# zijinxuxu/PDFNet

Measured on AMD Instinct MI355X. Metric: train-step images/sec @256x256 RGB-D B=32, higher is better.
Workload: dtype f32

## Files before the change

### include/pdfnet_hip.h

```cpp
#ifndef PDFNET_HIP_H
#define PDFNET_HIP_H
#ifdef __cplusplus
extern "C" {
#endif

#define PDF_E_BADARG (-1)
#define PDF_E_WORKSPACE (-2)
#define PDF_ACT_NONE 0
#define PDF_ACT_RELU 1
#define PDF_ACT_LRELU01 2


int pdf_linear_fwd(const float* x, const float* w, const float* bias, float* y,
                   int M, int N, int K, int ldx, int ldw, int ldy, int act, void* stream);
int pdf_linear_bwd_weight(const float* x, const float* dy, float* dw, float* db, float* ws, long ws_floats,
                          int M, int N, int K, int ldx, int lddy, int accumulate, void* stream);
long pdf_wgrad_workspace_floats(int M, int NI, int NJ);
int pdf_init(void);
int pdf_debug_init_device(void);
int pdf_debug_kernel_timing(int on);
int pdf_set_stats_output(float* part, long cap_floats);
long pdf_stats_result_tiles(void);
long pdf_stats_result_rows(void);
int pdf_set_bn_tile_stats(const float* part, long tiles, long rows_per_tile);
// ... 234 lines not shown
typedef struct PdfCallOpts {
    const void* op0_bf16; const void* op1_bf16;
    void* out_bf16;
    const void* bn_x_bf16;
    float* stats_out; long stats_cap;
    long stats_tiles; long stats_rows;
    const float* tile_stats; long tile_n; long tile_rows;
    const float* in_scale; const float* in_shift;
    const void* op1_bf16_t;
    float* ws; long ws_floats;
    const float* wino_v;
} PdfCallOpts;
long pdf_conv2d_winograd_v_offset(int N, int H, int W, int Cin, int Cout, int KH, int KW, int stride, int pad);
int pdf_linear_fwd_x(const float* x, const float* w, const float* bias, float* y, int M, int N, int K, int ldx, int ldw, int ldy, int act, void* stream, PdfCallOpts* opts);
int pdf_linear_fwd_pair_x(const float* x, const float* w0, const float* w1, const float* b0, const float* b1, float* y, int M, int N, int K, int ldx, int ldw, int ldy, int act, void* stream, PdfCallOpts* opts);
int pdf_linear_bwd_data_x(const float* dy, const float* w, float* dx, int M, int N, int K, int lddy, int ldw, int lddx, void* stream, PdfCallOpts* opts);
int pdf_linear_bwd_data_pair_x(const float* dy, const float* w0, const float* w1, float* dx, int M, int N, int K, int lddy, int ldw, int lddx, void* stream, PdfCallOpts* opts);
int pdf_conv2d_fwd_x(const float* x, const float* w, const float* bias, float* y, int N, int H, int W, int Cin, int ldx, int Cout, int KH, int KW, int stride, int pad, int OH, int OW, int ldy, int act, void* stream, PdfCallOpts* opts);
int pdf_conv2d_bwd_data_x(const float* dy, const float* w, float* dx, int N, int H, int W, int Cin, int lddx, int Cout, int KH, int KW, int stride, int pad, int OH, int OW, int lddy, void* stream, PdfCallOpts* opts);
int pdf_conv2d_bwd_data_add_x(const float* dy, const float* w, float* dx, int N, int H, int W, int Cin, int lddx, int Cout, int KH, int KW, int stride, int pad, int OH, int OW, int lddy, void* stream, PdfCallOpts* opts);
int pdf_linear_bwd_weight_x(const float* x, const float* dy, float* dw, float* db, float* ws, long ws_floats, int M, int N, int K, int ldx, int lddy, int accumulate, void* stream, PdfCallOpts* opts);
int pdf_linear_bwd_weight_pair_x(const float* x, const float* dy, float* dw0, float* dw1, float* db0, float* db1, float* ws, long ws_floats, int M, int N, int K, int ldx, int lddy, int accumulate, void* stream, PdfCallOpts* opts);
int pdf_conv2d_bwd_weight_x(const float* x, const float* dy, float* dw, float* db, float* ws, long ws_floats, int N, int H, int W, int Cin, int ldx, int Cout, int KH, int KW, int stride, int pad, int OH, int OW, int lddy, int accumulate, void* stream, PdfCallOpts* opts);
int pdf_deconv2d_fwd_x(const float* x, const float* w, const float* bias, float* y, int N, int H, int W, int Cin, int ldx, int Cout, int KH, int KW, int stride, int pad, int OH, int OW, int ldy, void* stream, PdfCallOpts* opts);
int pdf_deconv2d_bwd_data_x(const float* dy, const float* w, float* dx, int N, int H, int W, int Cin, int lddx, int Cout, int KH, int KW, int stride, int pad, int OH, int OW, int lddy, void* stream, PdfCallOpts* opts);
int pdf_deconv2d_bwd_weight_x(const float* x, const float* dy, float* dw, float* ws, long ws_floats, int N, int H, int W, int Cin, int ldx, int Cout, int KH, int KW, int stride, int pad, int OH, int OW, int lddy, int accumulate, void* stream, PdfCallOpts* opts);
int pdf_bn_train_fwd_x(const float* x, int ldx, int C, long R, const float* gamma, const float* beta, float* running_mean, float* running_var, float momentum, float eps, const float* res, int ldr, int relu, float* y, int ldy, float* save_mean, float* save_rstd, float* scale, float* shift, float* ws, void* stream, PdfCallOpts* opts);
int pdf_bn_train_bwd_x(const float* dy, int lddy, const float* y, int ldy, int relu, const float* x, int ldx, const float* save_mean, const float* save_rstd, const float* gamma, const float* scale, const float* shift, int C, long R, float* dx, int lddx, float* dres, int lddr, float* dgamma, float* dbeta, int accumulate, float* ws, void* stream, PdfCallOpts* opts);
int pdf_bn_relu_maxk_fwd_x(const float* y, int ldy, int C, long R, int K, const float* gamma, const float* beta, float* running_mean, float* running_var, float momentum, float eps, int training, float* out, int ldo, int* arg, float* save_mean, float* save_rstd, float* scale, float* shift, float* ws, void* stream, PdfCallOpts* opts);
int pdf_l2norm_cat_fwd_x(int nparts, const float* const* x, const int* C, const float* const* w, float eps, long R, float* y, int ldy, float* const* norm, void* stream, PdfCallOpts* opts);
long pdf_conv2d_winograd_workspace_floats(int N, int H, int W, int Cin, int Cout, int KH, int KW, int stride, int pad, int backward);
int pdf_debug_armed_slots(void);
int pdf_debug_callopts_size(void);

int pdf_x3_split(const float* x, void* out, long n, long cs, void* stream);
long pdf_deconv2d_x3_workspace_floats(int N, int H, int W, int Cin, int Cout, int KH, int KW, int stride, int pad, int backward);
int pdf_set_x3_mode(int mode);
int pdf_stream_create(void** out, int priority, int* lo, int* hi);
int pdf_debug_x3_mode(void);
int pdf_debug_x3_stamps(unsigned long long* out);
int pdf_x3_batched_gemm_nt(const void* A3, long csA, const void* B3, long csB, float* C, int batch, long gsA, long gsB, long gsC, int M, int N, int K, int variant, int nprod, void* stream);
int pdf_batched_gemm_nt(const float* A, const float* B, float* C, int batch, long gsA, long gsB, long gsC, int M, int N, int K, void* stream);
int pdf_x3_batched_gemm_tn(const void* P3, long csP, const void* Q3, long csQ, float* slab, int batch, long gsP, long gsQ, int M, int NI, int NJ, int splits, int variant, int nprod, void* stream);
int pdf_batched_gemm_tn(const float* P, const float* Q, float* slab, int batch, long gsP, long gsQ, int M, int NI, int NJ, int splits, void* stream);

typedef struct PdfMeshLin { const float* w[2]; const float* b[2]; } PdfMeshLin;
typedef struct PdfMeshLN { const float* g[2]; const float* b[2]; } PdfMeshLN;
typedef struct PdfMeshGcn { PdfMeshLin fc1, fc2, sc; PdfMeshLN n2, n3; unsigned long long seed; } PdfMeshGcn;
typedef struct PdfMeshAttn {
    PdfMeshLN ln; PdfMeshLin q, k, v, fc; PdfMeshLN ffln; PdfMeshLin f1, f2;
    unsigned long long seed_att, seed_z, seed_t, seed_x;
} PdfMeshAttn;
typedef struct PdfMeshLinG { float* w[2]; float* b[2]; } PdfMeshLinG;
typedef struct PdfMeshLNG { float* g[2]; float* b[2]; } PdfMeshLNG;
typedef struct PdfMeshGcnG { PdfMeshLinG fc1, fc2, sc; PdfMeshLNG n2, n3; } PdfMeshGcnG;
typedef struct PdfMeshAttnG { PdfMeshLNG ln; PdfMeshLinG q, k, v, fc; PdfMeshLNG ffln; PdfMeshLinG f1, f2; } PdfMeshAttnG;
typedef struct PdfMeshLevel {
    int level, B, training, cin0;
    float p;
    const unsigned long long* step;
    const float* x;
    float* out;
    const int* ell_col[2]; const float* ell_val[2]; const int* ell_colT[2]; const float* ell_valT[2]; int ell_w;
    PdfMeshGcn gcn[4];
    PdfMeshAttn self_, cross;
    float* tape;
    float* qkv;
    const float* dout;
    float* dx;
    float* gtape;
    PdfMeshGcnG ggcn[4]; PdfMeshAttnG gself, gcross;
    float* wg_ws; long wg_ws_floats;
} PdfMeshLevel;
long pdf_mesh_tape_floats(int level, int B);
long pdf_mesh_gtape_floats(int level, int B);
int pdf_mesh_level_fwd(const PdfMeshLevel* a, void* stream);
int pdf_mesh_level_bwd(const PdfMeshLevel* a, void* stream, void* side_stream);
int pdf_mesh_level_fwd_bf16(const PdfMeshLevel* a, void* stream);
int pdf_mesh_level_bwd_bf16(const PdfMeshLevel* a, void* stream, void* side_stream);
int pdf_mesh_level_fwd_x3(const PdfMeshLevel* a, void* stream);
int pdf_mesh_level_bwd_x3(const PdfMeshLevel* a, void* stream, void* side_stream);
int pdf_debug_mesh_level_size(void);

typedef struct PdfMeshLoss {
    const float* vp; const float* v2p; const float* hd3; const float* hd2; const float* r;
    const float* vgt[2]; const float* jgt[2]; const float* v2gt[2]; const float* lmsgt[2];
    const long long* ind; const float* K; const float* valid;
    const float* reg[2]; const long long* faces; const long long* perm[2];
    int B, Fc, size, down;
    float* part;
    float* out;
    float coef[12];
    const float* gmp;
    int edge_grad;
    float* dvp; float* dv2p; float* dhd3; float* dhd2; float* dr;
} PdfMeshLoss;
int pdf_mesh_loss_fwd(const PdfMeshLoss* a, void* stream);
int pdf_mesh_loss_bwd(const PdfMeshLoss* a, void* stream);
int pdf_debug_mesh_loss_size(void);
int pdf_debug_mesh_stamps(unsigned long long* out);

#ifdef __cplusplus
}
#endif
#endif
```

### pdfnet_amd/build.py

```python
import os
import subprocess
import sys
from concurrent.futures import ThreadPoolExecutor

HERE = os.path.dirname(os.path.abspath(__file__))
CSRC = os.path.join(HERE, "csrc")
LIB = os.path.join(HERE, "libpdfnet_hip.so")
INCLUDE = os.path.join(HERE, "..", "include")
SOURCES = ["gemm.hip", "gemm_dma.hip", "gemm_x3.hip", "winograd.hip", "gemm_bf16.hip", "pointops.hip", "norm.hip", "elementwise.hip", "graph.hip", "meshdec.hip", "meshdec_bf16.hip", "meshdec_x3.hip", "mano.hip", "frontend.hip", "loss.hip", "metrics.hip", "icp.hip", "meshcloud.hip", "penetration.hip", "silhouette.hip", "render.hip", "safused.hip"]
FLAGS = ["--offload-arch=gfx950", "-O3", "-fPIC", "-std=c++17", "-fvisibility=hidden", "-Wno-unused-result", "-I" + INCLUDE]


def _stale(target, deps):
    if not os.path.exists(target):
        return True
    t = os.path.getmtime(target)
    return any(os.path.getmtime(d) > t for d in deps)


def build(force=False, verbose=True):
    hipcc = os.environ.get("HIPCC", "/opt/rocm/bin/hipcc")
    hdrs = [os.path.join(CSRC, "common.h"), os.path.join(CSRC, "gemm_common.h"), os.path.join(CSRC, "gemm_internal.h"), os.path.join(CSRC, "svd3.h"), os.path.join(CSRC, "icp_common.h"), os.path.join(INCLUDE, "pdfnet_hip.h")]
    objs, jobs = [], []
    for s in SOURCES:
        src = os.path.join(CSRC, s)
        obj = os.path.join(CSRC, s.replace(".hip", ".o"))
        objs.append(obj)
        deps = [src] + hdrs + ([os.path.join(CSRC, "meshdec.hip")] if s in ("meshdec_bf16.hip", "meshdec_x3.hip") else [])
        if force or _stale(obj, deps):
            jobs.append([hipcc] + FLAGS + ["-c", src, "-o", obj])

    def run(cmd):
        if verbose:
            print(" ".join(cmd), flush=True)
        subprocess.check_call(cmd)
    with ThreadPoolExecutor(max_workers=4) as ex:
        list(ex.map(run, jobs))
    if force or jobs or _stale(LIB, objs):
        run([hipcc, "--offload-arch=gfx950", "-shared", "-fPIC", "-o", LIB] + objs)
    return LIB


if __name__ == "__main__":
    print(build(force="--force" in sys.argv))
```

### pdfnet_amd/functional.py

```python
import ctypes
import torch
from torch.autograd import Function

from . import hip
from .hip import ptr, ptr_at, stream

ACT_NONE, ACT_RELU, ACT_LRELU = 0, 1, 2
import os as _os

_byref = ctypes.byref
_CallOpts = hip.CallOpts
USE_SIDE_STREAMS = _os.environ.get("PDFNET_SIDE_STREAMS", "1") != "0"
_side = {}


def _record(obj, stream_):
    if torch.is_tensor(obj):
        obj.record_stream(stream_)
        s16 = getattr(obj, '_pdf_bf16', None)
        if s16 is not None:
            s16.record_stream(stream_)
    elif isinstance(obj, (list, tuple)):
        for o in obj:
            _record(o, stream_)
# ... 2646 lines not shown
                getattr(getattr(dst, k), wb)[hnd] = ptr(g)
        cur = stream()
        direct = all(g is None for g in grads)
        with wgrad_stream(direct, x, tape, qkv, gtape, ws, dout, params=tensors):
            _mesh_entry(L, 'bwd')(_byref(a), cur, stream())
        ctx.keep = ctx.args = None
        return (dx, None, None) + tuple(grads)


def mesh_level(layer, x):
    tensors, _ = _mesh_param_list(layer)
    return _MeshLevel.apply(x, layer, layer.training, *tensors)


def mesh_level_ok(layer, x):
    if not (MESH_FUSED and x.is_cuda and (MESH_FUSED_BF16 or not _GEMM_BF16) and x.dim() == 4 and x.shape[0] == 2 and x.dtype == torch.float32):
        return False
    level = {63: 0, 126: 1, 252: 2}.get(x.shape[2])
    return (level is not None and x.shape[3] == 2 * (256 >> level) and len(layer.graph_left.GCN_blocks) == 4 and layer.attn.n_heads == 4
            and layer.graph_left.GCN_blocks[0].fc1.weight.shape[0] == (256 >> level) and x.shape[1] <= 2048)


MESH_LOSS_FUSED = _os.environ.get("PDFNET_MESH_LOSS_FUSED", "1") != "0"
MESH_LOSS_TERMS = ('verts2d_loss', 'norm_loss', 'edge_loss', 'gcn_2d_loss', 'root_loss', 'verts_loss', 'abs_verts_loss', 'gcn_loss',
                   'abs_joints_loss', 'joints2d_loss', 'joints_loss', 'bone_direc_loss')


class _MeshLoss(Function):

    @staticmethod
    def forward(ctx, vp, v2p, hd3, hd2, r, gt, consts, size, down, edge_grad, coefs):
        hip.require_gpu(vp)
        vp, v2p, hd3, hd2, r = (t.contiguous() for t in (vp, v2p, hd3, hd2, r))
        B = vp.shape[1]
        if vp.shape[2:] != (778, 3) or hd3.shape[2:] != (252, 3):
            raise ValueError("pdfnet_amd: mesh_loss wants the decoder's 778- and 252-vertex meshes")
        a = hip.MeshLoss()
        keep = [vp, v2p, hd3, hd2, r]
        for k, t in (('vp', vp), ('v2p', v2p), ('hd3', hd3), ('hd2', hd2), ('r', r)):
            setattr(a, k, ptr(t))
        for k in ('vgt', 'jgt', 'v2gt', 'lmsgt'):
            for i in (0, 1):
                t = gt[k][i].contiguous()
                keep.append(t)
                getattr(a, k)[i] = ptr(t)
        for k in ('ind', 'K', 'valid'):
            t = gt[k].contiguous()
            keep.append(t)
            setattr(a, k, ptr(t))
        regs, faces, perms = consts
        a.reg[0], a.reg[1] = ptr(regs[0]), ptr(regs[1])
        a.faces = ptr(faces)
        a.perm[0], a.perm[1] = ptr(perms[0]), ptr(perms[1])
        a.B, a.Fc, a.size, a.down, a.edge_grad = B, faces.shape[1], int(size), int(down), 1 if edge_grad else 0
        for i, c in enumerate(coefs):
            a.coef[i] = float(c)
        part = torch.empty((2, B, 12), dtype=torch.float32, device=vp.device)
        out = torch.empty(4 + 9 * B, dtype=torch.float32, device=vp.device)
        a.part, a.out = ptr(part), ptr(out)
        _L().pdf_mesh_loss_fwd(_byref(a), stream())
        ctx.args, ctx.keep = a, keep + [regs, faces, perms, part]
        terms = out[:4 + 8 * B]
        ctx.mark_non_differentiable(terms)
        return out[4 + 8 * B:], terms

    @staticmethod
    def backward(ctx, g, _):
        a = ctx.args
        vp, v2p, hd3, hd2, r = ctx.keep[:5]
        g = g.contiguous()
        dvp, dv2p, dhd3, dhd2, dr = (torch.empty_like(t) for t in (vp, v2p, hd3, hd2, r))
        a.gmp = ptr(g)
        a.dvp, a.dv2p, a.dhd3, a.dhd2, a.dr = ptr(dvp), ptr(dv2p), ptr(dhd3), ptr(dhd2), ptr(dr)
        _L().pdf_mesh_loss_bwd(_byref(a), stream())
        return dvp, dv2p, dhd3, dhd2, dr, None, None, None, None, None, None


def mesh_loss(vp, v2p, hd3, hd2, r, gt, consts, size, down, edge_grad, coefs):
    mp, terms = _MeshLoss.apply(vp, v2p, hd3, hd2, r, gt, consts, size, down, edge_grad, tuple(coefs))
    B = vp.shape[1]
    d = {k: terms[i] for i, k in enumerate(MESH_LOSS_TERMS[:4])}
    d.update({k: terms[4 + i * B:4 + (i + 1) * B] for i, k in enumerate(MESH_LOSS_TERMS[4:])})
    return mp, d
```

### pdfnet_amd/hip.py

```python
import ctypes
import os
import re

import torch

_HERE = os.path.dirname(os.path.abspath(__file__))
LIB_PATH = os.environ.get("PDFNET_HIP_LIB") or os.path.join(_HERE, "libpdfnet_hip.so")
HEADER_PATH = os.path.join(_HERE, "..", "include", "pdfnet_hip.h")

_CT = {"int": ctypes.c_int, "long": ctypes.c_long, "float": ctypes.c_float,
       "unsigned long long": ctypes.c_ulonglong}


def _text(path):
    return re.sub(r"/\*.*?\*/", "", open(path).read(), flags=re.S)


def parse_header(path=HEADER_PATH):
    protos = {}
    for m in re.finditer(r"\b(int|long)\s+(pdf_\w+)\s*\(([^)]*)\)\s*;", _text(path)):
        ret, name, args = m.group(1), m.group(2), m.group(3)
        types = []
        for a in args.split(","):
            a = " ".join(a.split())
            if a in ("", "void"):
                continue
            if "*" in a:
                types.append(ctypes.c_void_p)
            else:
                base = a.rsplit(" ", 1)[0]
                types.append(_CT[base])
        protos[name] = (_CT[ret], types)
    return protos


def parse_structs(path=HEADER_PATH):
    txt, structs = _text(path), {}
    for m in re.finditer(r"typedef\s+struct\s+(\w+)\s*\{([^{}]*)\}\s*\1\s*;", txt):
        fields = []
        for decl in filter(None, (" ".join(d.split()) for d in m.group(2).split(";"))):
            try:
                first, *more = decl.split(",")
                base, star, name, dim = re.fullmatch(r"(?:const )?([\w ]+?) ?(\*?) ?(\w+)(?:\[(\d+)\])?", first).groups()
                ct = ctypes.c_void_p if star else _CT.get(base) or structs[base]
                names = [(name, dim)] + [re.fullmatch(r" ?(\w+)(?:\[(\d+)\])?", d).groups() for d in more]
                if star and more:
                    raise KeyError(decl)
            except (AttributeError, KeyError):
                raise ImportError("pdfnet_amd: %s: cannot bind field `%s` of %s" % (path, decl, m.group(1)))
            fields += [(n, ct * int(d) if d else ct) for n, d in names]
        structs[m.group(1)] = type(m.group(1), (ctypes.Structure,), {"_fields_": fields})
    if len(structs) != len(re.findall(r"\b(?:struct|union)\b[^;(]*\{", txt)):
        raise ImportError("pdfnet_amd: %s has a struct / union this binding cannot parse" % path)
    return structs


STRUCTS = parse_structs()
CallOpts, MeshLevel, MeshLoss = (STRUCTS[n] for n in ("PdfCallOpts", "PdfMeshLevel", "PdfMeshLoss"))


class _Lib:
    def __init__(self):
        if not os.path.exists(LIB_PATH):
            raise ImportError(
                "pdfnet_amd: %s is missing -- build it with `python -m pdfnet_amd.build` "
                "(hipcc --offload-arch=gfx950). There is no CPU or PyTorch fallback." % LIB_PATH)
        self.cdll = ctypes.CDLL(LIB_PATH)
        self.protos = parse_header()
        for name, (ret, args) in self.protos.items():
            fn = getattr(self.cdll, name)
            fn.restype = ret
            fn.argtypes = args
        for cls, fn in ((CallOpts, "pdf_debug_callopts_size"), (MeshLoss, "pdf_debug_mesh_loss_size"), (MeshLevel, "pdf_debug_mesh_level_size")):
            if getattr(self.cdll, fn)() != ctypes.sizeof(cls):
                raise ImportError("pdfnet_amd: %s of %s has %d bytes, this binding's has %d -- rebuild the library"
                                  % (cls.__name__, LIB_PATH, getattr(self.cdll, fn)(), ctypes.sizeof(cls)))

    def __getattr__(self, name):
        fn = getattr(self.cdll, name)
        is_status = self.protos[name][0] is ctypes.c_int and not name.startswith("pdf_debug_")

        def call(*args):
            rc = fn(*args)
            if is_status and rc != 0:
                raise RuntimeError("libpdfnet_hip: %s failed with code %d" % (name, rc))
            if _tape is not None and is_status:
                _tape.append((call, args))
            return rc
        setattr(self, name, call)
        return call


_lib = None
_tape = None


def lib():
    global _lib
    if _lib is None:
        _lib = _Lib()
        if torch.cuda.is_available():
            lr = os.environ.get("LOCAL_RANK")
            if lr is not None and torch.cuda.device_count() > 1 and int(lr) != torch.cuda.current_device():
                _lib = None
                raise RuntimeError("pdfnet_amd: LOCAL_RANK=%s but the current device is cuda:%d -- call torch.cuda.set_device(LOCAL_RANK) "
                                   "(trains.base_trainer.init_distributed) before the first pdfnet_amd call" % (lr, torch.cuda.current_device()))
            _lib.pdf_init()
    return _lib


def check_device(dev):
    L = lib()
    have = L.pdf_debug_init_device()
    idx = dev.index if dev.index is not None else torch.cuda.current_device()
    if have >= 0 and have != idx:
        raise RuntimeError("pdfnet_amd: libpdfnet_hip was initialised on cuda:%d, the model lives on cuda:%d (one process per GPU)" % (have, idx))


_raw_stream = getattr(torch._C, "_cuda_getCurrentRawStream", None)
_raw_device = getattr(torch._C, "_cuda_getDevice", None)


def stream():
    if _raw_stream is not None and _raw_device is not None:
        return _raw_stream(_raw_device())
    return torch.cuda.current_stream().cuda_stream


def ptr(t):
    return t.data_ptr() if t is not None else None


def ptr_at(t, elements):
    return t.data_ptr() + elements * t.element_size()


def require_gpu(*tensors):
    for t in tensors:
        if t is not None and not t.is_cuda:
            raise RuntimeError("pdfnet_amd ops run only on the GPU (HIP); got a %s tensor. "
                               "There is no CPU fallback in the product path." % t.device)
# ... 1 lines not shown
```

### pdfnet_amd/networks/intaghand_decoder.py

```python
import os

import numpy as np
import torch
import torch.nn as nn

from .. import functional as F
from .layers import Conv2d, Embedding, LayerNorm, Linear, xavier_

_DATA = os.path.join(os.path.dirname(os.path.abspath(__file__)), "..", "data", "gcn_core.npz")
IMG_SIZE = 384


def _csr_to_ell(indptr, indices, data, V):
    width = int(np.diff(indptr).max())
    col = np.zeros((V, width), np.int32)
    val = np.zeros((V, width), np.float32)
    for v in range(V):
        a, b = indptr[v], indptr[v + 1]
        col[v, :b - a] = indices[a:b]
        val[v, :b - a] = data[a:b]
    return col, val


def load_graph_constants():
# ... 165 lines not shown
        self.position_embeddings = Embedding(V, cin)
        self.graph_left = GraphLayer(cin, cout, ellL, n, drop)
        self.graph_right = GraphLayer(cin, cout, ellR, n, drop)
        self.img_ex_left = img_ex(img_size, img_c, 6, grid_c, cout, heads, drop)
        self.img_ex_right = img_ex(img_size, img_c, 6, grid_c, cout, heads, drop)
        self.attn = inter_attn(cout, heads, drop)

    def forward(self, x):
        x = x + self.position_embeddings.weight
        if F.mesh_level_ok(self, x):
            return F.mesh_level(self, x)
        blocks = list(zip(self.graph_left.GCN_blocks, self.graph_right.GCN_blocks))
        for i, (bl, br) in enumerate(blocks):
            x = gcn_block_pair(bl, br, x, relu_out=i != len(blocks) - 1)
        return self.attn(x)


class DualGraph(nn.Module):
    def __init__(self, layers):
        super().__init__()
        self.layers = nn.ModuleList(layers)

    def forward(self, x):
        last = len(self.layers) - 1
        for i, layer in enumerate(self.layers):
            x = layer(x)
            if i != last:
                x = x.repeat_interleave(2, dim=2)
        return x


def projection_batch(scale, trans2d, pts, img_size):
    s = (scale * img_size).view(-1, 1, 1)
    t = (trans2d * img_size / 2 + img_size / 2).unsqueeze(1)
    return s * pts[..., :2] + t


class decoder(nn.Module):
    def __init__(self, opt, dropout=0.05, num_attn_heads=4):
        super().__init__()
        g = load_graph_constants()
        self.register_buffer('dense_coor', g['dense_coor'].clone())
        for h in ('left', 'right'):
            self.register_buffer('graph_perm_' + h, g['perm_' + h].clone(), persistent=False)
            self.register_buffer('graph_perm_reverse_' + h, g['perm_rev_' + h].clone(), persistent=False)
        self.converter = {h: GCN_vert_convert(self, h) for h in ('left', 'right')}
        cin, cout = opt.GCN_IN_DIM, opt.GCN_OUT_DIM
        layers = []
        for i, V in enumerate((63, 126, 252)):
            layers.append(DualGraphLayer(V, cin[i], cout[i], g['ell_left'][i], g['ell_right'][i], opt.graph_layer_num,
                                         [12, 24, 48][i], opt.DECONV_DIMS[i], opt.IMG_DIMS[i], num_attn_heads, dropout))
        self.dual_gcn = DualGraph(layers)
        d0 = cin[0] - 3
        self.gf_layer_left = nn.Sequential(Linear(1024, d0), LayerNorm(d0))
        self.gf_layer_right = nn.Sequential(Linear(1024, d0), LayerNorm(d0))
        self.unsample_layer = Linear(252, 778, bias=False)
        self.unsample_layer.weight.data.copy_(g['upsample'])
        self.coord_head = Linear(cout[-1], 3)
        self.avg_head = Linear(252, 1)
        self.params_head = Linear(cout[-1], 3)
        self.root_head = Linear(cout[-1], 3)
        for m in (self.gf_layer_left, self.gf_layer_right, self.coord_head, self.avg_head, self.params_head, self.root_head):
            xavier_(m)
        self._pe_key, self._pe = None, None

    def get_converter(self):
        return self.converter

    def hand_pe(self):
        key = (self.dense_coor._version, self.dense_coor.device)
        if self._pe_key != key:
            with torch.no_grad():
                c = (self.dense_coor * 2 - 1).unsqueeze(0)
                self._pe = torch.stack([self.converter[h].vert_to_GCN(c).view(1, 63, 16, 3).mean(2) for h in ('left', 'right')])
            self._pe_key = key
        return self._pe

    def forward(self, gl, gr):
        bs = gl.shape[0]
        g = torch.stack((gl, gr))
        f = _ln2(self.gf_layer_left[1], self.gf_layer_right[1], _lin2(self.gf_layer_left[0], self.gf_layer_right[0], g))
        x = torch.cat([f.unsqueeze(2).expand(-1, -1, 63, -1), self.hand_pe().expand(-1, bs, -1, -1)], -1)
        x = self.dual_gcn(x)
        t = self.avg_head(x.transpose(2, 3))[..., 0]
        p = self.params_head(t)
        rt = self.root_head(t)
        c3 = self.coord_head(x)
        up3 = self.unsample_layer(c3.transpose(2, 3)).transpose(2, 3).contiguous()
        sc, tr = p[..., 0], p[..., 1:]
        c2 = projection_batch(sc.reshape(-1), tr.reshape(-1, 2), c3.reshape(2 * bs, -1, 3), IMG_SIZE).view(2, bs, -1, 2)
        up2 = projection_batch(sc.reshape(-1), tr.reshape(-1, 2), up3.reshape(2 * bs, -1, 3), IMG_SIZE).view(2, bs, -1, 2)
        hands = ('left', 'right')
        scale = {h: sc[i] for i, h in enumerate(hands)}
        trans2d = {h: tr[i] for i, h in enumerate(hands)}
        root = {h: rt[i] for i, h in enumerate(hands)}
        v3 = {h: c3[i] for i, h in enumerate(hands)}
        v2 = {h: c2[i] for i, h in enumerate(hands)}
        result = {'verts3d': {h: up3[i] for i, h in enumerate(hands)}, 'verts2d': {h: up2[i] for i, h in enumerate(hands)}}
        other = {'verts3d_MANO_list': {'left': [], 'right': []}, 'verts2d_MANO_list': {'left': [], 'right': []}}
        for hand in hands:
            for key, src in (('verts3d_MANO_list', v3), ('verts2d_MANO_list', v2)):
                other[key][hand].append(self.converter[hand].GCN_to_vert(src[hand].repeat_interleave(4, dim=1)))
        return (result, {'scale': scale, 'trans2d': trans2d, 'root': root},
                [{'verts3d': v3, 'verts2d': v2}], other)


def load_decoder(opt, encoder_info=None):
    return decoder(opt, dropout=0.05, num_attn_heads=4)
```

Baseline: 718.7.

## Fuse decoder tail heads, upsample and projection into custom HIP kernels

Replaces the decoder tail (avg head, params/root/coord heads, 252→778 upsample, and both 2D projections) with one forward kernel per hand-batch item, plus a fused backward kernel and a finish kernel that reduces weight gradients across the batch. It targets the many small launches and intermediate tensors of the original chain of linear layers and transposes. In exchange, shapes are hardcoded (252 vertices, 64 channels, 778 upsampled), and the per-block backward uses large shared memory with one block per hand-batch item, so the grid is only 64 blocks.

Measured after the change: 721.2 (median of 6 runs). Within noise of the previous version (+0.4%).

```diff
diff --git a/include/pdfnet_hip.h b/include/pdfnet_hip.h
--- a/include/pdfnet_hip.h
+++ b/include/pdfnet_hip.h
@@ -340,6 +340,17 @@
 int pdf_mesh_level_bwd_x3(const PdfMeshLevel* a, void* stream, void* side_stream);
 int pdf_debug_mesh_level_size(void);
 
+#define PDF_MESH_TAIL_PART 840
+int pdf_mesh_tail_fwd(int B, float img_size, const float* x, const float* avg_w, const float* avg_b, const float* par_w, const float* par_b,
+                      const float* root_w, const float* root_b, const float* coord_w, const float* coord_b, const float* up_w,
+                      float* t, float* p, float* rt, float* c3, float* up3, float* c2, float* up2, void* stream);
+int pdf_mesh_tail_bwd(int B, float img_size, const float* x, const float* t, const float* p, const float* c3, const float* up3,
+                      const float* avg_w, const float* par_w, const float* root_w, const float* coord_w, const float* up_w,
+                      const float* dp, const float* drt, const float* dc3, const float* dup3, const float* dc2, const float* dup2,
+                      float* dx, float* gup, float* part,
+                      float* g_avg_w, float* g_avg_b, float* g_par_w, float* g_par_b, float* g_root_w, float* g_root_b, float* g_coord_w, float* g_coord_b,
+                      float* g_up_w, int overwrite, void* stream);
+
 typedef struct PdfMeshLoss {
     const float* vp; const float* v2p; const float* hd3; const float* hd2; const float* r;
     const float* vgt[2]; const float* jgt[2]; const float* v2gt[2]; const float* lmsgt[2];
diff --git a/pdfnet_amd/build.py b/pdfnet_amd/build.py
--- a/pdfnet_amd/build.py
+++ b/pdfnet_amd/build.py
@@ -7,7 +7,7 @@
 CSRC = os.path.join(HERE, "csrc")
 LIB = os.path.join(HERE, "libpdfnet_hip.so")
 INCLUDE = os.path.join(HERE, "..", "include")
-SOURCES = ["gemm.hip", "gemm_dma.hip", "gemm_x3.hip", "winograd.hip", "gemm_bf16.hip", "pointops.hip", "norm.hip", "elementwise.hip", "graph.hip", "meshdec.hip", "meshdec_bf16.hip", "meshdec_x3.hip", "mano.hip", "frontend.hip", "loss.hip", "metrics.hip", "icp.hip", "meshcloud.hip", "penetration.hip", "silhouette.hip", "render.hip", "safused.hip"]
+SOURCES = ["gemm.hip", "gemm_dma.hip", "gemm_x3.hip", "winograd.hip", "gemm_bf16.hip", "pointops.hip", "norm.hip", "elementwise.hip", "graph.hip", "meshdec.hip", "meshdec_bf16.hip", "meshdec_x3.hip", "meshglue.hip", "mano.hip", "frontend.hip", "loss.hip", "metrics.hip", "icp.hip", "meshcloud.hip", "penetration.hip", "silhouette.hip", "render.hip", "safused.hip"]
 FLAGS = ["--offload-arch=gfx950", "-O3", "-fPIC", "-std=c++17", "-fvisibility=hidden", "-Wno-unused-result", "-I" + INCLUDE]
 
 
diff --git a/pdfnet_amd/csrc/meshglue.hip b/pdfnet_amd/csrc/meshglue.hip
--- /dev/null
+++ b/pdfnet_amd/csrc/meshglue.hip
@@ -0,0 +1,354 @@
+#include "common.h"
+
+#define MT_T 1024
+#define MT_V 252
+#define MT_C 64
+#define MT_U 778
+#define MT_LDX 65
+#define MT_PART PDF_MESH_TAIL_PART
+#define MT_P_CW 0
+#define MT_P_CB 192
+#define MT_P_PW 195
+#define MT_P_PB 387
+#define MT_P_RW 390
+#define MT_P_RB 582
+#define MT_P_AW 585
+#define MT_P_AB 837
+#define MT_P_END 838
+static_assert(MT_P_END <= MT_PART, "PDF_MESH_TAIL_PART is too small");
+
+#define MT_FWD_SMEM (MT_V * MT_LDX + 1024 + 1024 + 64 + 192 + 8)
+#define MT_BWD_SMEM (MT_V * MT_LDX + 16 * MT_V * 3 + 1024 + MT_U * 4 + 64 + 64 + 192 + 64)
+
+struct MeshTail {
+    int B;
+    float img_size;
+    const float* x;
+    const float *avg_w, *avg_b, *par_w, *par_b, *root_w, *root_b, *coord_w, *coord_b, *up_w;
+    float *t, *p, *rt, *c3, *up3, *c2, *up2;
+    const float *dp, *drt, *dc3, *dup3, *dc2, *dup2;
+    float *dx, *gup, *part;
+    float *g_avg_w, *g_avg_b, *g_par_w, *g_par_b, *g_root_w, *g_root_b, *g_coord_w, *g_coord_b, *g_up_w;
+    int overwrite;
+};
+
+__device__ __forceinline__ void mt_load_x(const float* __restrict__ x, float* xs, int tid) {
+    for (int i = tid; i < MT_V * MT_C / 4; i += MT_T) {
+        const float4 v = reinterpret_cast<const float4*>(x)[i];
+        float* d = xs + (i >> 4) * MT_LDX + (i & 15) * 4;
+        d[0] = v.x; d[1] = v.y; d[2] = v.z; d[3] = v.w;
+    }
+}
+
+__global__ __launch_bounds__(MT_T, 1) void mesh_tail_fwd_kernel(const MeshTail a) {
+    extern __shared__ float smem[];
+    float* xs = smem;
+    float* red = xs + MT_V * MT_LDX;
+    float* c3s = red + 1024;
+    float* ts = c3s + 1024;
+    float* wcs = ts + 64;
+    float* ps = wcs + 192;
+    const int tid = threadIdx.x, lane = tid & 63, w = tid >> 6;
+    const long hb = blockIdx.x;
+    mt_load_x(a.x + hb * MT_V * MT_C, xs, tid);
+    if (tid < 192) wcs[tid] = a.coord_w[tid];
+    __syncthreads();
+    {
+        float s = 0.f;
+        for (int v = w; v < MT_V; v += 16) s += a.avg_w[v] * xs[v * MT_LDX + lane];
+        red[w * 64 + lane] = s;
+    }
+    if (tid < MT_V * 3) {
+        const int v = tid / 3, j = tid - 3 * v;
+        float s = a.coord_b[j];
+        const float* xr = xs + v * MT_LDX;
+        const float* wr = wcs + j * 64;
+#pragma unroll 16
+        for (int c = 0; c < MT_C; ++c) s += wr[c] * xr[c];
+        c3s[v * 4 + j] = s;
+        a.c3[(hb * MT_V + v) * 3 + j] = s;
+    }
+    __syncthreads();
+    if (tid < 64) {
+        float s = a.avg_b[0];
+#pragma unroll
+        for (int q = 0; q < 16; ++q) s += red[q * 64 + tid];
+        ts[tid] = s;
+        a.t[hb * 64 + tid] = s;
+    }
+    __syncthreads();
+    if (w < 6) {
+        const int j = w % 3;
+        const float s = wave_sum((w < 3 ? a.par_w : a.root_w)[j * 64 + lane] * ts[lane]) + (w < 3 ? a.par_b : a.root_b)[j];
+        if (lane == 0) {
+            ps[w] = s;
+            (w < 3 ? a.p : a.rt)[hb * 3 + j] = s;
+        }
+    }
+    __syncthreads();
+    const float sc = ps[0] * a.img_size;
+    const float tx = ps[1] * a.img_size / 2.f + a.img_size / 2.f, ty = ps[2] * a.img_size / 2.f + a.img_size / 2.f;
+    if (tid < MT_V) {
+        a.c2[(hb * MT_V + tid) * 2 + 0] = sc * c3s[tid * 4 + 0] + tx;
+        a.c2[(hb * MT_V + tid) * 2 + 1] = sc * c3s[tid * 4 + 1] + ty;
+    }
+    float cx[4], cy[4], cz[4];
+#pragma unroll
+    for (int k = 0; k < 4; ++k) {
+        const int v = lane + 64 * k;
+        const bool ok = v < MT_V;
+        cx[k] = ok ? c3s[v * 4 + 0] : 0.f;
+        cy[k] = ok ? c3s[v * 4 + 1] : 0.f;
+        cz[k] = ok ? c3s[v * 4 + 2] : 0.f;
+    }
+    for (int u0 = w; u0 < MT_U; u0 += 64) {
+        float uw[4][4];
+#pragma unroll
+        for (int r = 0; r < 4; ++r) {
+            const int u = u0 + 16 * r;
+#pragma unroll
+            for (int k = 0; k < 4; ++k) {
+                const int v = lane + 64 * k;
+                uw[r][k] = (u < MT_U && v < MT_V) ? a.up_w[(long)u * MT_V + v] : 0.f;
+            }
+        }
+#pragma unroll
+        for (int r = 0; r < 4; ++r) {
+            const int u = u0 + 16 * r;
+            float s0 = 0.f, s1 = 0.f, s2 = 0.f;
+#pragma unroll
+            for (int k = 0; k < 4; ++k) { s0 += uw[r][k] * cx[k]; s1 += uw[r][k] * cy[k]; s2 += uw[r][k] * cz[k]; }
+            s0 = wave_sum(s0); s1 = wave_sum(s1); s2 = wave_sum(s2);
+            if (lane == 0 && u < MT_U) {
+                float* o3 = a.up3 + (hb * MT_U + u) * 3;
+                o3[0] = s0; o3[1] = s1; o3[2] = s2;
+                float* o2 = a.up2 + (hb * MT_U + u) * 2;
+                o2[0] = sc * s0 + tx; o2[1] = sc * s1 + ty;
+            }
+        }
+    }
+}
+
+__global__ __launch_bounds__(MT_T, 1) void mesh_tail_bwd_kernel(const MeshTail a) {
+    extern __shared__ float smem[];
+    float* xs = smem;
+    float* red = xs + MT_V * MT_LDX;
+    float* d3s = red + 16 * MT_V * 3;
+    float* gs = d3s + 1024;
+    float* dts = gs + MT_U * 4;
+    float* tss = dts + 64;
+    float* wcs = tss + 64;
+    float* sm = wcs + 192;
+    const int tid = threadIdx.x, lane = tid & 63, w = tid >> 6;
+    const long hb = blockIdx.x;
+    const float sc = a.p[hb * 3] * a.img_size;
+    float ds = 0.f, d1 = 0.f, d2 = 0.f;
+    if (tid < MT_U) {
+        const long o = hb * MT_U + tid;
+        float g0 = 0.f, g1 = 0.f, g2 = 0.f;
+        if (a.dup3 != nullptr) { g0 = a.dup3[o * 3]; g1 = a.dup3[o * 3 + 1]; g2 = a.dup3[o * 3 + 2]; }
+        if (a.dup2 != nullptr) {
+            const float e0 = a.dup2[o * 2], e1 = a.dup2[o * 2 + 1];
+            g0 += sc * e0; g1 += sc * e1;
+            ds = e0 * a.up3[o * 3] + e1 * a.up3[o * 3 + 1];
+            d1 = e0; d2 = e1;
+        }
+        gs[tid * 4 + 0] = g0; gs[tid * 4 + 1] = g1; gs[tid * 4 + 2] = g2; gs[tid * 4 + 3] = 0.f;
+        a.gup[o * 3] = g0; a.gup[o * 3 + 1] = g1; a.gup[o * 3 + 2] = g2;
+    }
+    if (tid < MT_V && a.dc2 != nullptr) {
+        const long o = hb * MT_V + tid;
+        const float e0 = a.dc2[o * 2], e1 = a.dc2[o * 2 + 1];
+        ds += e0 * a.c3[o * 3] + e1 * a.c3[o * 3 + 1];
+        d1 += e0; d2 += e1;
+    }
+    ds = wave_sum(ds); d1 = wave_sum(d1); d2 = wave_sum(d2);
+    if (lane == 0) { sm[w * 3] = ds; sm[w * 3 + 1] = d1; sm[w * 3 + 2] = d2; }
+    mt_load_x(a.x + hb * MT_V * MT_C, xs, tid);
+    if (tid < 192) wcs[tid] = a.coord_w[tid];
+    if (tid < 64) tss[tid] = a.t[hb * 64 + tid];
+    __syncthreads();
+    if (lane < 63) {
+        float s[4][3] = {};
+#pragma unroll 7
+        for (int u = w; u < MT_U; u += 16) {
+            const float4 uw = *reinterpret_cast<const float4*>(a.up_w + (long)u * MT_V + lane * 4);
+            const float4 g = *reinterpret_cast<const float4*>(gs + u * 4);
+            s[0][0] += uw.x * g.x; s[0][1] += uw.x * g.y; s[0][2] += uw.x * g.z;
+            s[1][0] += uw.y * g.x; s[1][1] += uw.y * g.y; s[1][2] += uw.y * g.z;
+            s[2][0] += uw.z * g.x; s[2][1] += uw.z * g.y; s[2][2] += uw.z * g.z;
+            s[3][0] += uw.w * g.x; s[3][1] += uw.w * g.y; s[3][2] += uw.w * g.z;
+        }
+        float* r = red + (w * MT_V + lane * 4) * 3;
+#pragma unroll
+        for (int k = 0; k < 4; ++k) { r[k * 3] = s[k][0]; r[k * 3 + 1] = s[k][1]; r[k * 3 + 2] = s[k][2]; }
+    }
+    __syncthreads();
+    if (tid < MT_V * 3) {
+        const int v = tid / 3, j = tid - 3 * v;
+        float d = 0.f;
+#pragma unroll
+        for (int q = 0; q < 16; ++q) d += red[(q * MT_V + v) * 3 + j];
+        const long o = hb * MT_V + v;
+        if (a.dc3 != nullptr) d += a.dc3[o * 3 + j];
+        if (a.dc2 != nullptr && j < 2) d += sc * a.dc2[o * 2 + j];
+        d3s[v * 4 + j] = d;
+    } else if (tid >= 768 && tid < 774) {
+        const int k = tid - 768, j = k % 3;
+        float val;
+        if (k < 3) {
+            float s = 0.f;
+#pragma unroll
+            for (int q = 0; q < 16; ++q) s += sm[q * 3 + j];
+            val = s * (j == 0 ? a.img_size : a.img_size / 2.f);
+            if (a.dp != nullptr) val += a.dp[hb * 3 + j];
+        } else {
+            val = a.drt != nullptr ? a.drt[hb * 3 + j] : 0.f;
+        }
+        sm[48 + k] = val;
+    }
+    __syncthreads();
+    float* part = a.part + hb * MT_PART;
+    if (w == 0) {
+        float s = 0.f;
+#pragma unroll
+        for (int j = 0; j < 3; ++j) s += a.par_w[j * 64 + lane] * sm[48 + j] + a.root_w[j * 64 + lane] * sm[51 + j];
+        dts[lane] = s;
+        s = wave_sum(s);
+        if (lane == 0) part[MT_P_AB] = s;
+    } else if (w < 4) {
+        const int j = w - 1;
+        float s = 0.f;
+#pragma unroll
+        for (int k = 0; k < 4; ++k) s += lane + 64 * k < MT_V ? d3s[(lane + 64 * k) * 4 + j] : 0.f;
+        s = wave_sum(s);
+        if (lane == 0) part[MT_P_CB + j] = s;
+    }
+    __syncthreads();
+    if (tid < 768) {
+        const int o = tid % 192, q = tid / 192, j = o >> 6, c = o & 63;
+        float s = 0.f;
+#pragma unroll 9
+        for (int v = q; v < MT_V; v += 4) s += d3s[v * 4 + j] * xs[v * MT_LDX + c];
+        red[q * 192 + o] = s;
+    } else if (tid - 768 < MT_V) {
+        const int v = tid - 768;
+        float s = 0.f;
+        const float* xr = xs + v * MT_LDX;
+#pragma unroll 16
+        for (int c = 0; c < MT_C; ++c) s += dts[c] * xr[c];
+        part[MT_P_AW + v] = s;
+    }
+    for (int i = tid; i < 384; i += MT_T) {
+        const int k = i >> 6, c = i & 63;
+        part[(k < 3 ? MT_P_PW : MT_P_RW - 192) + i] = sm[48 + k] * tss[c];
+    }
+    if (tid < 6) part[(tid < 3 ? MT_P_PB : MT_P_RB - 3) + tid] = sm[48 + tid];
+    float* dx = a.dx + hb * MT_V * MT_C;
+    for (int i = tid; i < MT_V * MT_C; i += MT_T) {
+        const int v = i >> 6, c = i & 63;
+        dx[i] = d3s[v * 4] * wcs[c] + d3s[v * 4 + 1] * wcs[64 + c] + d3s[v * 4 + 2] * wcs[128 + c] + a.avg_w[v] * dts[c];
+    }
+    __syncthreads();
+    if (tid < 192) part[MT_P_CW + tid] = red[tid] + red[192 + tid] + red[384 + tid] + red[576 + tid];
+}
+
+__device__ __forceinline__ void mt_put(float* g, int i, float s, bool overwrite) {
+    if (g != nullptr) g[i] = overwrite ? s : g[i] + s;
+}
+
+#define MT_FIN_BLOCKS (MT_U + (MT_P_END + 63) / 64)
+__global__ __launch_bounds__(1024) void mesh_tail_finish_kernel(const MeshTail a) {
+    __shared__ float red[1024];
+    const int tid = threadIdx.x, nhb = 2 * a.B;
+    if (blockIdx.x < MT_U) {
+        if (a.g_up_w == nullptr) return;
+        const int u = blockIdx.x, v = tid & 255, q = tid >> 8;
+        float s = 0.f;
+        if (v < MT_V) {
+#pragma unroll 8
+            for (long hb = (long)q * nhb / 4; hb < (long)(q + 1) * nhb / 4; ++hb) {
+                const float* g = a.gup + (hb * MT_U + u) * 3;
+                const float* c = a.c3 + (hb * MT_V + v) * 3;
+                s += g[0] * c[0] + g[1] * c[1] + g[2] * c[2];
+            }
+        }
+        red[tid] = s;
+        __syncthreads();
+        if (tid < MT_V) mt_put(a.g_up_w, u * MT_V + tid, red[tid] + red[256 + tid] + red[512 + tid] + red[768 + tid], (a.overwrite >> 8) & 1);
+        return;
+    }
+    const int i = (blockIdx.x - MT_U) * 64 + (tid & 63), q = tid >> 6;
+    float s = 0.f;
+    if (i < MT_P_END) {
+#pragma unroll 4
+        for (long hb = (long)q * nhb / 16; hb < (long)(q + 1) * nhb / 16; ++hb) s += a.part[hb * MT_PART + i];
+    }
+    red[tid] = s;
+    __syncthreads();
+    if (tid < 64 && i < MT_P_END) {
+        s = 0.f;
+#pragma unroll
+        for (int k = 0; k < 16; ++k) s += red[k * 64 + tid];
+        if (i < MT_P_CB) mt_put(a.g_coord_w, i - MT_P_CW, s, (a.overwrite >> 6) & 1);
+        else if (i < MT_P_PW) mt_put(a.g_coord_b, i - MT_P_CB, s, (a.overwrite >> 7) & 1);
+        else if (i < MT_P_PB) mt_put(a.g_par_w, i - MT_P_PW, s, (a.overwrite >> 2) & 1);
+        else if (i < MT_P_RW) mt_put(a.g_par_b, i - MT_P_PB, s, (a.overwrite >> 3) & 1);
+        else if (i < MT_P_RB) mt_put(a.g_root_w, i - MT_P_RW, s, (a.overwrite >> 4) & 1);
+        else if (i < MT_P_AW) mt_put(a.g_root_b, i - MT_P_RB, s, (a.overwrite >> 5) & 1);
+        else if (i < MT_P_AB) mt_put(a.g_avg_w, i - MT_P_AW, s, (a.overwrite >> 0) & 1);
+        else mt_put(a.g_avg_b, 0, s, (a.overwrite >> 1) & 1);
+    }
+}
+
+PDF_API int pdf_mesh_tail_fwd(int B, float img_size, const float* x, const float* avg_w, const float* avg_b, const float* par_w, const float* par_b,
+                              const float* root_w, const float* root_b, const float* coord_w, const float* coord_b, const float* up_w,
+                              float* t, float* p, float* rt, float* c3, float* up3, float* c2, float* up2, void* stream) {
+    if (B < 1 || B > (1 << 20) || x == nullptr || avg_w == nullptr || avg_b == nullptr || par_w == nullptr || par_b == nullptr || root_w == nullptr ||
+        root_b == nullptr || coord_w == nullptr || coord_b == nullptr || up_w == nullptr) return PDF_E_BADARG;
+    if (t == nullptr || p == nullptr || rt == nullptr || c3 == nullptr || up3 == nullptr || c2 == nullptr || up2 == nullptr) return PDF_E_BADARG;
+    if ((reinterpret_cast<uintptr_t>(x) & 15) != 0) return PDF_E_BADARG;
+    MeshTail a = {};
+    a.B = B; a.img_size = img_size; a.x = x;
+    a.avg_w = avg_w; a.avg_b = avg_b; a.par_w = par_w; a.par_b = par_b; a.root_w = root_w; a.root_b = root_b; a.coord_w = coord_w; a.coord_b = coord_b; a.up_w = up_w;
+    a.t = t; a.p = p; a.rt = rt; a.c3 = c3; a.up3 = up3; a.c2 = c2; a.up2 = up2;
+    const size_t smem = (size_t)MT_FWD_SMEM * sizeof(float);
+    static bool attr_done = false;
+    if (!attr_done) {
+        if (hipError_t e = hipFuncSetAttribute(reinterpret_cast<const void*>(mesh_tail_fwd_kernel), hipFuncAttributeMaxDynamicSharedMemorySize, (int)smem)) return (int)e;
+        attr_done = true;
+    }
+    hipLaunchKernelGGL(mesh_tail_fwd_kernel, dim3(2 * B), dim3(MT_T), smem, (hipStream_t)stream, a);
+    PDF_LAUNCH_CHECK();
+    return 0;
+}
+
+PDF_API int pdf_mesh_tail_bwd(int B, float img_size, const float* x, const float* t, const float* p, const float* c3, const float* up3,
+                              const float* avg_w, const float* par_w, const float* root_w, const float* coord_w, const float* up_w,
+                              const float* dp, const float* drt, const float* dc3, const float* dup3, const float* dc2, const float* dup2,
+                              float* dx, float* gup, float* part,
+                              float* g_avg_w, float* g_avg_b, float* g_par_w, float* g_par_b, float* g_root_w, float* g_root_b, float* g_coord_w, float* g_coord_b,
+                              float* g_up_w, int overwrite, void* stream) {
+    if (B < 1 || B > (1 << 20) || x == nullptr || t == nullptr || p == nullptr || c3 == nullptr || up3 == nullptr || avg_w == nullptr || par_w == nullptr ||
+        root_w == nullptr || coord_w == nullptr || up_w == nullptr || dx == nullptr || gup == nullptr || part == nullptr) return PDF_E_BADARG;
+    if ((reinterpret_cast<uintptr_t>(x) & 15) != 0) return PDF_E_BADARG;
+    MeshTail a = {};
+    a.B = B; a.img_size = img_size; a.x = x;
+    a.t = const_cast<float*>(t); a.p = const_cast<float*>(p); a.c3 = const_cast<float*>(c3); a.up3 = const_cast<float*>(up3);
+    a.avg_w = avg_w; a.par_w = par_w; a.root_w = root_w; a.coord_w = coord_w; a.up_w = up_w;
+    a.dp = dp; a.drt = drt; a.dc3 = dc3; a.dup3 = dup3; a.dc2 = dc2; a.dup2 = dup2;
+    a.dx = dx; a.gup = gup; a.part = part;
+    a.g_avg_w = g_avg_w; a.g_avg_b = g_avg_b; a.g_par_w = g_par_w; a.g_par_b = g_par_b; a.g_root_w = g_root_w; a.g_root_b = g_root_b;
+    a.g_coord_w = g_coord_w; a.g_coord_b = g_coord_b; a.g_up_w = g_up_w; a.overwrite = overwrite;
+    const size_t smem = (size_t)MT_BWD_SMEM * sizeof(float);
+    static bool attr_done = false;
+    if (!attr_done) {
+        if (hipError_t e = hipFuncSetAttribute(reinterpret_cast<const void*>(mesh_tail_bwd_kernel), hipFuncAttributeMaxDynamicSharedMemorySize, (int)smem)) return (int)e;
+        attr_done = true;
+    }
+    hipLaunchKernelGGL(mesh_tail_bwd_kernel, dim3(2 * B), dim3(MT_T), smem, (hipStream_t)stream, a);
+    PDF_LAUNCH_CHECK();
+    hipLaunchKernelGGL(mesh_tail_finish_kernel, dim3(MT_FIN_BLOCKS), dim3(1024), 0, (hipStream_t)stream, a);
+    PDF_LAUNCH_CHECK();
+    return 0;
+}
diff --git a/pdfnet_amd/functional.py b/pdfnet_amd/functional.py
--- a/pdfnet_amd/functional.py
+++ b/pdfnet_amd/functional.py
@@ -2752,3 +2752,64 @@
     d = {k: terms[i] for i, k in enumerate(MESH_LOSS_TERMS[:4])}
     d.update({k: terms[4 + i * B:4 + (i + 1) * B] for i, k in enumerate(MESH_LOSS_TERMS[4:])})
     return mp, d
+
+
+MESH_GLUE = _os.environ.get("PDFNET_MESH_GLUE", "1") != "0"
+
+
+def mesh_tail_ok(dec, x):
+    return (MESH_GLUE and x.is_cuda and not _GEMM_BF16 and x.dtype == torch.float32 and x.dim() == 4 and x.shape[0] == 2 and x.shape[2:] == (252, 64)
+            and dec.unsample_layer.weight.shape == (778, 252) and dec.unsample_layer.bias is None and dec.avg_head.weight.shape == (1, 252)
+            and all(m.weight.shape == (3, 64) for m in (dec.params_head, dec.root_head, dec.coord_head)))
+
+
+def _mesh_tail_params(dec):
+    return (dec.avg_head.weight, dec.avg_head.bias, dec.params_head.weight, dec.params_head.bias, dec.root_head.weight, dec.root_head.bias,
+            dec.coord_head.weight, dec.coord_head.bias, dec.unsample_layer.weight)
+
+
+class _MeshTail(Function):
+
+    @staticmethod
+    def forward(ctx, x, img_size, *params):
+        hip.require_gpu(x)
+        if not x.is_contiguous():
+            raise ValueError("pdfnet_amd: mesh_tail wants the level's contiguous output")
+        B, dev = x.shape[1], x.device
+        new = lambda *s: torch.empty((2, B) + s, dtype=torch.float32, device=dev)
+        t, p, rt, c3, up3, c2, up2 = new(64), new(3), new(3), new(252, 3), new(778, 3), new(252, 2), new(778, 2)
+        if not all(w.is_contiguous() for w in params):
+            raise ValueError("pdfnet_amd: mesh_tail wants contiguous parameters")
+        _L().pdf_mesh_tail_fwd(B, float(img_size), ptr(x), *(ptr(w) for w in params), *(ptr(o) for o in (t, p, rt, c3, up3, c2, up2)), stream())
+        if any(ctx.needs_input_grad):
+            ctx.set_materialize_grads(False)
+            ctx.img_size, ctx.keep, ctx.params = float(img_size), (x, t, p, c3, up3), params
+        return p, rt, c3, up3, c2, up2
+
+    @staticmethod
+    def backward(ctx, dp, drt, dc3, dup3, dc2, dup2):
+        (x, t, p, c3, up3), params = ctx.keep, ctx.params
+        B = x.shape[1]
+        ups = [None if g is None else g.contiguous() for g in (dp, drt, dc3, dup3, dc2, dup2)]
+        dx = torch.empty_like(x)
+        gup = torch.empty((2, B, 778, 3), dtype=torch.float32, device=x.device)
+        part = torch.empty((2, B, hip.MESH_TAIL_PART), dtype=torch.float32, device=x.device)
+        grads, dst, over = [], [], 0
+        for i, w in enumerate(params):
+            g = ret = None
+            if ctx.needs_input_grad[2 + i]:
+                g = _main_grad(w, w)
+                if g is None:
+                    g = ret = torch.empty_like(w)
+                    over |= 1 << i
+            dst.append(g)
+            grads.append(ret)
+        avg_w, _, par_w, _, root_w, _, coord_w, _, up_w = params
+        _L().pdf_mesh_tail_bwd(B, ctx.img_size, ptr(x), ptr(t), ptr(p), ptr(c3), ptr(up3), ptr(avg_w), ptr(par_w), ptr(root_w), ptr(coord_w), ptr(up_w),
+                               *(ptr(g) for g in ups), ptr(dx), ptr(gup), ptr(part), *(ptr(g) for g in dst), over, stream())
+        ctx.keep = ctx.params = None
+        return (dx, None) + tuple(grads)
+
+
+def mesh_tail(dec, x, img_size):
+    return _MeshTail.apply(x, img_size, *_mesh_tail_params(dec))
diff --git a/pdfnet_amd/hip.py b/pdfnet_amd/hip.py
--- a/pdfnet_amd/hip.py
+++ b/pdfnet_amd/hip.py
@@ -57,6 +57,7 @@
 
 STRUCTS = parse_structs()
 CallOpts, MeshLevel, MeshLoss = (STRUCTS[n] for n in ("PdfCallOpts", "PdfMeshLevel", "PdfMeshLoss"))
+MESH_TAIL_PART = int(re.search(r"#define\s+PDF_MESH_TAIL_PART\s+(\d+)", _text(HEADER_PATH)).group(1))
 
 
 class _Lib:
diff --git a/pdfnet_amd/networks/intaghand_decoder.py b/pdfnet_amd/networks/intaghand_decoder.py
--- a/pdfnet_amd/networks/intaghand_decoder.py
+++ b/pdfnet_amd/networks/intaghand_decoder.py
@@ -271,14 +271,22 @@
         f = _ln2(self.gf_layer_left[1], self.gf_layer_right[1], _lin2(self.gf_layer_left[0], self.gf_layer_right[0], g))
         x = torch.cat([f.unsqueeze(2).expand(-1, -1, 63, -1), self.hand_pe().expand(-1, bs, -1, -1)], -1)
         x = self.dual_gcn(x)
-        t = self.avg_head(x.transpose(2, 3))[..., 0]
-        p = self.params_head(t)
-        rt = self.root_head(t)
-        c3 = self.coord_head(x)
-        up3 = self.unsample_layer(c3.transpose(2, 3)).transpose(2, 3).contiguous()
-        sc, tr = p[..., 0], p[..., 1:]
-        c2 = projection_batch(sc.reshape(-1), tr.reshape(-1, 2), c3.reshape(2 * bs, -1, 3), IMG_SIZE).view(2, bs, -1, 2)
-        up2 = projection_batch(sc.reshape(-1), tr.reshape(-1, 2), up3.reshape(2 * bs, -1, 3), IMG_SIZE).view(2, bs, -1, 2)
+        return self.tail(x)
+
+    def tail(self, x):
+        bs = x.shape[1]
+        if F.mesh_tail_ok(self, x):
+            p, rt, c3, up3, c2, up2 = F.mesh_tail(self, x, IMG_SIZE)
+            sc, tr = p[..., 0], p[..., 1:]
+        else:
+            t = self.avg_head(x.transpose(2, 3))[..., 0]
+            p = self.params_head(t)
+            rt = self.root_head(t)
+            c3 = self.coord_head(x)
+            up3 = self.unsample_layer(c3.transpose(2, 3)).transpose(2, 3).contiguous()
+            sc, tr = p[..., 0], p[..., 1:]
+            c2 = projection_batch(sc.reshape(-1), tr.reshape(-1, 2), c3.reshape(2 * bs, -1, 3), IMG_SIZE).view(2, bs, -1, 2)
+            up2 = projection_batch(sc.reshape(-1), tr.reshape(-1, 2), up3.reshape(2 * bs, -1, 3), IMG_SIZE).view(2, bs, -1, 2)
         hands = ('left', 'right')
         scale = {h: sc[i] for i, h in enumerate(hands)}
         trans2d = {h: tr[i] for i, h in enumerate(hands)}
```
